# mayataka/idocp

Measured on AMD Instinct MI355X. Metric: SQP iterations/sec (whole node), higher is better.
Workload: dtype f64; 1 GPU; ANYmal OCPSolver N=100 T=5.05 FP64, trotting contact sequence (1 lift + 9 impulse events, 120 stages incl. impulse / aux / lift stages, switching constraints; BASELINE.json configs[2]); batch=1024 independent OCP instances per GPU, replicas across GPUs; horizon=100, batch_per_gpu=1024, parallelism=replicas x1

## Files before the change

idocp_amd/csrc/ocp_condense_kernel.hip:

```cpp
#include <hip/hip_runtime.h>

#include <cstdlib>

#include "dev_dense.hpp"
#include "dev_lie.hpp"
#include "dev_rnea_tangent.hpp"
#include "ocp_device.hpp"
#include "ocp_launch.hpp"

namespace idocp_dev {

#ifdef IDOCP_K5_TILES16
#define K5_TILE_PAIR mfmaTilePairTN
#else
#define K5_TILE_PAIR mfmaTilePairTN4
#endif

__device__ __forceinline__ double ocpLimit(const OcpProblem* __restrict__ P, int comp, int r) {
  switch (comp) {
    case 0: return P->q_min[r];
    case 1: return P->q_max[r];
    case 2: return -P->v_max[r];
    case 3: return P->v_max[r];
    case 4: return -P->u_max[r];
// ... 464 lines not shown
        for (int m = 0; m < 6; ++m) acc += sm[S::BL + r + SF * m] * sm[GG + c + SF * m];
#pragma unroll
        for (int m = 0; m < NJ; ++m) acc += sm[TT + r + SF * m] * sm[S::JM + c + SF * (6 + m)];
        sm[S::SM + r + SF * c] = acc;
      }
      waveLdsSync();
      if (dimf > 0) {
        constexpr int WW = (TT + SF * NJ + SF * SF <= S::VEC) ? TT + SF * NJ : S::WSM;
        static_assert(WW != S::WSM || !S::SEP_MINV, "the narrow layouts keep W behind G and Jl D^-1");
        spdInverseCholDpp<SF>(&sm[S::SM], SF, dimf, lane, &s_ok, &sm[WW], SF);
      }
    } else {
      ldsFlagWait(&s_gt, 1, lane);
      ldsFlagWait(&s_ba, 3, lane);
      for (int e = lane; e < dimf * NJ; e += 64) {
        const int c = e / dimfd, r = e - c * dimfd;
        double acc = sm[TT + r + SF * c];
#pragma unroll
        for (int m = 0; m < 6; ++m) acc += sm[GG + r + SF * m] * sm[S::MINV + m + NV * (6 + c)];
        sm[S::BL + r + SF * (6 + c)] = acc;
      }
    }
    STAMPW(3);
  }
  blockLdsBarrier();
  STAMP(2);
  if (MERIT) {
    rneaAssembleNominal<D>(tid, sc, out);
    blockLdsBarrier();
    if (!impulse && tid >= 6 && tid < NV && nd->has_u) sm[S::IDC + tid] -= s_g[L::S_U + tid - 6];
    blockLdsBarrier();
    if (tid < dimvf) merit_viol += dt * fabs(sm[S::IDC + tid]);
    if (sw_dimi > 0 && tid >= 200 && tid < 200 + sw_dimi) merit_viol += fabs(B.swc[rec * L::SWC + L::W_P + tid - 200]);
    blockLdsBarrier();
    sm[S::ERR + tid] = merit_cost; sm[S::ERR + nt + tid] = merit_viol;
    blockLdsBarrier();
    if (tid < 2) {
      double e = 0.0;
      for (int t = 0; t < nt; ++t) e += sm[S::ERR + nt * tid + t];
      if (B.ext) e += B.ext[rec * L::EXT + (tid == 1 ? L::X_VIOL : L::X_COST)];
      B.merit_stage[rec * 4 + tid] = e;
    }
    return;
  }
  STAMP(5);
  asm volatile("" : "+v"(tid) :: "memory");
  if (RESIDUAL) {
    rneaAssembleQV<D>(bwp, tid, nt, sc, out);
    blockLdsBarrier();
    if (!impulse && tid >= 6 && tid < NV && nd->has_u) sm[S::IDC + tid] -= s_g[L::S_U + tid - 6];
    blockLdsBarrier();
    if (tid >= 128 && tid < 128 + NV) {
      const int r = tid - 128;
      const double dq = dotAny(&sm[S::DIDC + SVF * r], 1, &sm[S::BM], 1, dimvf);
      const double dv = dotAny(&sm[S::DIDC + SVF * (NV + r)], 1, &sm[S::BM], 1, dimvf);
      const double da = dotAny(&sm[S::MM + NV * r], 1, &sm[S::BM], 1, NV) + dotAny(&sm[S::JM + SF * r], 1, &sm[S::BM + NV], 1, dimf);
      const double lq = sm[S::LQ + r] + dt * dq, lv = sm[S::LV + r] + dt * dv, la = sm[S::LA + r] + dt * da;
      const double idr = sm[S::IDC + r];
      err_local += lq * lq + lv * lv + la * la + dt * dt * idr * idr;
    } else if (tid >= 192 && tid < 192 + NC) {
      const int c = tid - 192;
      if (nd->active[c]) {
        const int row = nd->row_of[c];
        for (int x = 0; x < 3; ++x) {
          double jb = 0.0;
          for (int col = 0; col < NV; ++col) jb += sm[S::JM + (row + x) + SF * col] * sm[S::BM + col];
          const double lf = sm[S::LF + row + x] - dt * jb;
          const double cr = sm[S::IDC + NV + row + x];
          err_local += lf * lf + dt * dt * cr * cr;
        }
      }
    }
    if (sw_dimi > 0 && tid >= 200 && tid < 200 + sw_dimi) {
      const double pr = B.swc[rec * L::SWC + L::W_P + tid - 200];
      err_local += pr * pr;
    }
    blockLdsBarrier();
    sm[S::ERR + tid] = err_local + (BWD ? 1.0 : dt * dt) * err_ipm;
    blockLdsBarrier();
    if (tid == 0) {
      double e = 0.0;
      for (int t = 0; t < nt; ++t) e += sm[S::ERR + t];
      if (B.ext) e += (BWD ? 1.0 : dt * dt) * B.ext[rec * L::EXT + L::X_ERR];
      B.err_stage[rec] = e;
    }
    return;
  }
  constexpr bool EARLY_MJ = (SVF * SVF <= RS::FEET);
  auto assembleTR = [&]() {
    for (int e = tid; e < dimf * NV; e += nt) {
      const int c = e / NV, r = e - c * NV;
      const double tr = dotAny(&sm[S::BL + SF * r], 1, &sm[S::SM + SF * c], 1, dimf);
      sm[S::MJ + r + SVF * (NV + c)] = tr;
      sm[S::MJ + (NV + c) + SVF * r] = tr;
    }
    for (int e = tid; e < dimf * dimf; e += nt) { const int c = e / dimfd, r = e - c * dimfd; sm[S::MJ + (NV + r) + SVF * (NV + c)] = -sm[S::SM + r + SF * c]; }
  };
  STAMPW(7);
  rneaAssembleQV<D>(bwp, tid, nt, sc, out);
  STAMPW(5);
  if (tid >= 160 && tid < 160 + NV) sm[S::LA + tid - 160] += dt * sm[S::TLA + tid - 160];
  if (tid >= 128 && tid < 128 + 6) {
    const int r = tid - 128;
    double acc = 0.0;
    for (int m2 = 0; m2 < 6; ++m2) acc += sm[S::FQQI + r + 6 * m2] * sm[S::FQ + m2];
    sm[S::FQ6 + r] = BWD ? acc : -acc;
  }
  if constexpr (EARLY_MJ) assembleTR();
  STAMPW(6);
  blockLdsBarrier();
  if (tid < dimvf) {
    double val = sm[S::IDC + tid];
    if (!impulse && tid >= 6 && tid < NV && nd->has_u) { val -= s_g[L::S_U + tid - 6]; sm[S::IDC + tid] = val; }
    sm[S::DIDC + tid + SVF * NX] = val;
  }
  if (tid >= 64 && tid < 64 + 6) sm[S::FQ + tid - 64] = sm[S::FQ6 + tid - 64];
  if constexpr (!EARLY_MJ) {
    assembleTR();
    blockLdsBarrier();
  }
  STAMP(6);
  for (int e = tid; e < NV * NV; e += nt) {
    const int c = e / NV, r = e - c * NV;
    sm[S::MJ + r + SVF * c] = sm[S::MINV + e] - dotAny(&sm[S::MJ + r + SVF * NV], SVF, &sm[S::BL + SF * c], 1, dimf);
  }
  {
    const int part = tid & 3;
    double acc = 0.0;
    int dst = -1;
    double sgn = dt;
    if (tid < 4 * NX) {
      const int g = tid >> 2;
      const int q4 = (dimvf + 3) >> 2, k0 = part * q4, k1 = (k0 + q4 < dimvf) ? k0 + q4 : dimvf;
      const double* col = &sm[S::DIDC + SVF * g];
      for (int k = k0; k < k1; ++k) acc += col[k] * sm[S::BM + k];
      dst = (g < NV) ? S::LQ + g : S::LV + g - NV;
    } else if (tid >= 160 && tid < 160 + 4 * SF) {
      const int r = (tid - 160) >> 2;
      if (r < dimf) {
        constexpr int q4 = (NV + 3) / 4;
        const int k0 = part * q4, k1 = (k0 + q4 < NV) ? k0 + q4 : NV;
        for (int col = k0; col < k1; ++col) acc += sm[S::JM + r + SF * col] * sm[S::BM + col];
        dst = S::LF + r; sgn = -dt;
      }
    }
    acc += __shfl_xor(acc, 1);
    acc += __shfl_xor(acc, 2);
    if (part == 0 && dst >= 0) sm[dst] += sgn * acc;
  }
  blockLdsBarrier();

  const double hu = (PLAIN || nd->has_u) ? 1.0 : 0.0;
  STAMP(7);
  {
    const int wave = tid >> 6, lane = tid & 63;
    constexpr int TX = (NX + 15) / 16;
    static_assert(RVF <= 32, "two row tiles");
    for (int jb = wave; jb < TX; jb += nt >> 6) {
      mfma_d4 a0, a1;
      const int r1 = dimvf > 16 ? dimvf - 16 : 1;
      K5_TILE_PAIR<RVF>(&sm[S::MJ], dimvf < 16 ? dimvf : 16, &sm[S::DIDC + SVF * 16 * jb], NX + 1 - 16 * jb, &sm[S::MJ + SVF * 16], r1,
                          &sm[S::DIDC + SVF * 16 * jb], NX + 1 - 16 * jb, SVF, SVF, dimvf, lane, a0, a1);
      auto put = [&](int r, int c, double v) { sm[S::MJD + r + SVF * c] = v; };
      mfmaTileStore(a0, 0, 16 * jb, dimvf, NX + 1, lane, put);
      mfmaTileStore(a1, 16, 16 * jb, dimvf, NX + 1, lane, put);
    }
  }
  STAMP(11);
  const double* const mjidc = &sm[S::MJD + SVF * NX];
#pragma unroll
  for (int t = 0; t < (NV * NV + nt - 1) / nt; ++t) {
    const int e = tid + nt * t;
    if (e < NV * NV) { const int c = e / NV, r = e - c * NV; sm[S::QAFU + r + SVF * c] = hu * sm[S::QAA + r] * sm[S::MJ + r + SVF * c]; }
  }
  for (int e = tid; e < dimf * NV; e += nt) {
    const int c = e / dimfd, r = e - c * dimfd;
    sm[S::QAFU + NV + r + SVF * c] = hu * dotAny(&sm[S::QFF + r], SF, &sm[S::MJ + NV + SVF * c], 1, dimf);
  }
  STAMP(12);
  blockLdsBarrier();
  STAMP(13);
#pragma unroll
  for (int t = 0; t < (NV * NX + nt - 1) / nt; ++t) {
    const int e = tid + nt * t;
    if (e < NV * NX) { const int c = e / NV, r = e - c * NV; sm[S::QAFQV + r + SVF * c] = -sm[S::QAA + r] * sm[S::MJD + r + SVF * c]; }
  }
  for (int e = tid; e < dimf * NX; e += nt) {
    const int c = e / dimfd, r = e - c * dimfd;
    sm[S::QAFQV + NV + r + SVF * c] = -dotAny(&sm[S::QFF + r], SF, &sm[S::MJD + NV + SVF * c], 1, dimf);
  }
  if (tid < dimvf) {
    const int r = tid;
    double val;
    if (r < NV) val = sm[S::LA + r] - sm[S::QAA + r] * mjidc[r];
    else { double acc = 0.0; for (int p = 0; p < dimf; ++p) acc += sm[S::QFF + (r - NV) + SF * p] * mjidc[NV + p]; val = -sm[S::LF + r - NV] - acc; }
    sm[S::LAF + r] = val;
  }
  blockLdsBarrier();
  STAMP(8);
  {
    const int wave = tid >> 6, lane = tid & 63;
    constexpr int NJOB = 14;
    static_assert(NX <= 48 && NV <= 32 && NU <= 16, "tile counts of the job list");
    auto operands = [&](int j, const double*& X, int& xr, const double*& Y, int& yc, int& r0, int& c0) {
      if (j < 6) {
        const int ib = j < 3 ? 0 : (j < 5 ? 1 : 2), jb = j < 3 ? j : (j < 5 ? j - 2 : 2);
        X = &sm[S::MJD + SVF * 16 * ib]; xr = NX - 16 * ib; Y = &sm[S::QAFQV + SVF * 16 * jb]; yc = NX - 16 * jb; r0 = 16 * ib; c0 = 16 * jb;
      } else if (j < 12) {
        const int ib = (j - 6) >> 1, jb = (j - 6) & 1;
        X = &sm[S::MJD + SVF * 16 * ib]; xr = NX - 16 * ib; Y = &sm[S::QAFU + SVF * 16 * jb]; yc = NV - 16 * jb; r0 = 16 * ib; c0 = 16 * jb;
      } else {
        const int ib = j - 12;
        X = &sm[S::MJ + SVF * 16 * ib]; xr = NV - 16 * ib; Y = &sm[S::QAFU + SVF * 6]; yc = NU; r0 = 16 * ib; c0 = 0;
      }
    };
    auto finish = [&](int j, const mfma_d4& acc, int r0, int c0) {
      const int r = r0 + (lane & 15), g4 = lane >> 4;
      if (j < 6) {
        double b6[4];
        const double dg = sm[S::HQD + (r < NX ? r : NX - 1)];
        static_assert(S::HVD == S::HQD + NV, "one diagonal vector");
#pragma unroll
        for (int q = 0; q < 4; ++q) { const int c = c0 + g4 + 4 * q; b6[q] = sm[S::QB6 + (r < 6 ? r : 5) + 6 * (c < 6 ? c : 5)]; }
#pragma unroll
        for (int q = 0; q < 4; ++q) {
          const int c = c0 + g4 + 4 * q;
          const double base = (r < 6 && c < 6) ? b6[q] : (r == c ? dg : 0.0);
          if (r <= c && c < NX) kk[L::K_QXX + L::xsym(r, c)] = base - acc[q];
        }
      } else if (j < 12) {
#pragma unroll
        for (int q = 0; q < 4; ++q) {
          const int c = c0 + g4 + 4 * q;
          double* dst = c < 6 ? ee + (L::E_QXUP + r + NX * c) : kk + (L::K_QXU + r + NX * (c - 6));
          if (r < NX && c < NV) *dst = -acc[q];
        }
      } else {
        double hd[4];
#pragma unroll
        for (int q = 0; q < 4; ++q) { const int c = c0 + g4 + 4 * q; hd[q] = sm[S::HUD + (c < NU ? c : NU - 1)]; }
#pragma unroll
        for (int q = 0; q < 4; ++q) {
          const int c = c0 + g4 + 4 * q;
          double* dst = r < 6 ? ee + (L::E_QUUP + r + 6 * c) : kk + (L::K_QUU + (r - 6) + NU * c);
          const double v = acc[q] + ((r >= 6 && r - 6 == c) ? hd[q] : 0.0);
          if (r < NV && c < NU) *dst = v;
        }
      }
    };
    auto pair = [&](auto jc) {
      constexpr int j = decltype(jc)::value;
      const double *X0, *Y0, *X1, *Y1;
      int xr0, yc0, r00, c00, xr1, yc1, r01, c01;
      operands(j, X0, xr0, Y0, yc0, r00, c00);
      operands(j + 1, X1, xr1, Y1, yc1, r01, c01);
      mfma_d4 a0, a1;
      K5_TILE_PAIR<RVF>(X0, xr0, Y0, yc0, X1, xr1, Y1, yc1, SVF, SVF, dimvf, lane, a0, a1);
      finish(j, a0, r00, c00);
      finish(j + 1, a1, r01, c01);
    };
    static_assert(nt == 256 && NJOB == 14, "four wavefronts: jobs 2 w, 2 w + 1 and 2 w + 8, 2 w + 9");
    switch (__builtin_amdgcn_readfirstlane(wave)) {
      case 0: pair(std::integral_constant<int, 0>{}); pair(std::integral_constant<int, 8>{}); break;
      case 1: pair(std::integral_constant<int, 2>{}); pair(std::integral_constant<int, 10>{}); break;
      case 2: pair(std::integral_constant<int, 4>{}); pair(std::integral_constant<int, 12>{}); break;
      default: pair(std::integral_constant<int, 6>{}); break;
    }
  }
  STAMP(14);
  {
    const int part = tid & 3, g = tid >> 2;
    const int q4 = (dimvf + 3) >> 2, k0 = part * q4, k1 = (k0 + q4 < dimvf) ? k0 + q4 : dimvf;
    double acc = 0.0;
    if (g < NX) { const double* col = &sm[S::MJD + SVF * g]; for (int k = k0; k < k1; ++k) acc += col[k] * sm[S::LAF + k]; }
    else if (g < NX + NV) { const double* row = &sm[S::MJ + (g - NX)]; for (int k = k0; k < k1; ++k) acc += row[SVF * k] * sm[S::LAF + k]; }
    acc += __shfl_xor(acc, 1);
    acc += __shfl_xor(acc, 2);
    if (part == 0) {
      if (g < NV) sm[S::LQ + g] -= acc;
      else if (g < NX) sm[S::LV + g - NV] -= acc;
      else if (g < NX + NV) {
        const int r = g - NX;
        if (r < 6) sm[S::LUP + r] += hu * acc; else sm[S::LU + r - 6] += hu * acc;
        sm[S::FV + r] -= dt * mjidc[r];
      }
    }
  }
  static_assert(4 * (NX + NV) <= nt, "a quad per row of the vector updates");
  blockLdsBarrier();

  STAMP(9);
  typedef double wd2 __attribute__((ext_vector_type(2)));
  static_assert(NV % 2 == 0 && SVF % 2 == 0 && S::MJD % 2 == 0 && L::K_FVQ % 2 == 0 && L::K_FVV % 2 == 0 && L::KKT % 2 == 0, "16-byte stores of Fvq / Fvv");
  for (int e = tid; e < NV * NV / 2; e += nt) {
    const int c = e / (NV / 2), r = 2 * (e - c * (NV / 2));
    const wd2 mq = *reinterpret_cast<const wd2*>(&sm[S::MJD + r + SVF * c]), mvv = *reinterpret_cast<const wd2*>(&sm[S::MJD + r + SVF * (NV + c)]);
    const double one = BWD ? -1.0 : 1.0;
    wd2 fq, fv;
    fq.x = -dt * mq.x; fq.y = -dt * mq.y;
    fv.x = -dt * mvv.x + (r == c ? one : 0.0); fv.y = -dt * mvv.y + (r + 1 == c ? one : 0.0);
    *reinterpret_cast<wd2*>(&kk[L::K_FVQ + r + NV * c]) = fq;
    *reinterpret_cast<wd2*>(&kk[L::K_FVV + r + NV * c]) = fv;
  }
  for (int e = tid; e < NV * NU; e += nt) { const int c = e / NV, r = e - c * NV; kk[L::K_FVU + e] = hu * dt * sm[S::MJ + r + SVF * (6 + c)]; }
  if (tid < NV) {
    kk[L::K_LX + tid] = sm[S::LQ + tid]; kk[L::K_LX + NV + tid] = sm[S::LV + tid];
    kk[L::K_FX + tid] = sm[S::FQ + tid]; kk[L::K_FX + NV + tid] = sm[S::FV + tid];
  }
  if (tid < NU) kk[L::K_LU + tid] = sm[S::LU + tid];
  for (int t = tid; t < RVF * (RVF + 1) / 2; t += nt) {
    const int pr = t / (RVF + 1), idx = t - pr * (RVF + 1);
    const bool lo = idx <= pr;
    const int r = lo ? pr : RVF - 1 - pr, c = lo ? idx : idx - pr - 1;
    ee[L::E_MJ + r * (r + 1) / 2 + c] = sm[S::MJ + r + SVF * c];
  }
  static_assert(RVF % 2 == 0 && NVF % 2 == 0 && L::E_MJD % 2 == 0 && L::EXP % 2 == 0, "16-byte stores of MJtJinv_dIDCdqv");
  for (int e = tid; e < (RVF / 2) * NX; e += nt) {
    const int c = e / (RVF / 2), r = 2 * (e - c * (RVF / 2));
    *reinterpret_cast<wd2*>(&ee[L::E_MJD + r + NVF * c]) = *reinterpret_cast<const wd2*>(&sm[S::MJD + r + SVF * c]);
  }
  if (tid < NV) ee[L::E_QAA + tid] = sm[S::QAA + tid];
  for (int e = tid; e < SF * SF; e += nt) { const int c = e / SF, r = e - c * SF; ee[L::E_QFF + r + NF * c] = sm[S::QFF + e]; }
  if (tid < RVF) { ee[L::E_MJIDC + tid] = mjidc[tid]; ee[L::E_LAF + tid] = sm[S::LAF + tid]; }
  if (tid < 6) ee[L::E_LUP + tid] = sm[S::LUP + tid];
  if (sw_dimi > 0) {
    const int dimi = sw_dimi;
    double* __restrict__ W = B.swc + rec * L::SWC;
    for (int e = tid; e < dimi * NX; e += nt) {
      const int c = e / dimi, j = e - c * dimi;
      double acc = 0.0;
      for (int m2 = 0; m2 < NV; ++m2) acc += W[L::W_PHIA + j + NF * m2] * sm[S::MJD + m2 + SVF * c];
      W[L::W_PHIX + j + NF * c] -= acc;
    }
    for (int e = tid; e < dimi * NU; e += nt) {
      const int c = e / dimi, j = e - c * dimi;
      double acc = 0.0;
      for (int m2 = 0; m2 < NV; ++m2) acc += W[L::W_PHIA + j + NF * m2] * sm[S::MJ + m2 + SVF * (6 + c)];
      W[L::W_PHIU + j + NF * c] = acc;
    }
    if (tid < dimi) {
      double acc = 0.0;
      for (int m2 = 0; m2 < NV; ++m2) acc += W[L::W_PHIA + tid + NF * m2] * mjidc[m2];
      W[L::W_P + tid] -= acc;
    }
  }
  STAMP(10);
  if (tid == 0 && !s_ok && B.status[b] == 0) B.status[b] = 1 + pos;
  };
  stage((long)blockIdx.x);
#undef STAMP
#undef STAMPW
}


template <typename D>
__global__ __launch_bounds__(64) void parnmpc_lie_kernel(OcpBuffers B, const double* __restrict__ q0) {
  using L = OcpLayout<D>;
  constexpr int NQ = D::NQ;
  const OcpProblem* __restrict__ P = B.prob;
  const int M = B.M;
  const long unit = (long)blockIdx.x * 64 + threadIdx.x;
  if (unit >= (long)P->batch * (M - 1)) return;
  const long b = unit / (M - 1);
  const int pos = (int)(unit - b * (M - 1));
  const OcpNode* __restrict__ nd = B.nodes + pos;
  const int task = blockIdx.y;
  const long rec = b * B.NS + nd->slot;
  const double* __restrict__ s = B.sol + rec * L::SOL;
  const double* __restrict__ q = s + L::S_Q;
  double* __restrict__ zz = B.lie + rec * L::LIE;
  double R[9], p[3], Ja[36], Jb[36], d6[6];
  if (task == 0) {
    lieRelative(B.q_ref + (long)pos * NQ, q, R, p);
    lieLog6(R, p, d6);
    lieJlog6(R, p, Ja);
    for (int k = 0; k < 36; ++k) zz[L::Z_JQ + k] = Ja[k];
    for (int k = 0; k < 6; ++k) zz[L::Z_QDIFF + k] = d6[k];
  } else if (task == 1) {
    lieRelative(B.sol + (b * B.NS + nd->next) * L::SOL + L::S_Q, q, R, p);
    lieJlog6(R, p, Ja);
    for (int k = 0; k < 36; ++k) zz[L::Z_FQQ + k] = Ja[k];
  } else {
    const double* __restrict__ q_prev = (nd->prev < 0) ? (q0 + b * NQ) : (B.sol + (b * B.NS + nd->prev) * L::SOL + L::S_Q);
    lieRelative(q, q_prev, R, p);
    lieLog6(R, p, d6);
    for (int k = 0; k < 6; ++k) zz[L::Z_FQ6 + k] = d6[k];
    lieJlog6(R, p, Ja);
    lieDDiffArg0(R, p, Ja, Jb);
    for (int k = 0; k < 36; ++k) zz[L::Z_FQQP + k] = Jb[k];
    lieBlockInverse(Ja, Jb);
    for (int k = 0; k < 36; ++k) zz[L::Z_FQQI + k] = Jb[k];
  }
}

template <typename D>
static void launchCondense(const OcpBuffers& B, long batch, int M, int dimf, const double* q0, hipStream_t st, bool residual, int part = 0) {
  const size_t smem = CondenseSmem<D>::TOTAL * sizeof(double);
  static bool configured = false;
  if (!configured) {
    (void)hipFuncSetAttribute((const void*)ocp_condense_kernel<D, false, -1>, hipFuncAttributeMaxDynamicSharedMemorySize, (int)smem);
    (void)hipFuncSetAttribute((const void*)ocp_condense_kernel<D, false, -1, false, false, true>, hipFuncAttributeMaxDynamicSharedMemorySize, (int)smem);
    (void)hipFuncSetAttribute((const void*)ocp_condense_kernel<D, false, D::NF>, hipFuncAttributeMaxDynamicSharedMemorySize, (int)smem);
    (void)hipFuncSetAttribute((const void*)ocp_condense_kernel<D, false, D::NF, false, false, true>, hipFuncAttributeMaxDynamicSharedMemorySize, (int)smem);
    (void)hipFuncSetAttribute((const void*)ocp_condense_kernel<D, true, -1>, hipFuncAttributeMaxDynamicSharedMemorySize, (int)smem);
    configured = true;
  }
  const unsigned blocks = (unsigned)(batch * M);
  if (part != 2) {
    OcpLaunch<D>::nominal(B, batch, M, st, q0);
    OcpLaunch<D>::extRows(B, batch, M, residual, st);
  }
  if (part == 1) return;
  if (residual) hipLaunchKernelGGL((ocp_condense_kernel<D, true, -1>), dim3(blocks), dim3(256), smem, st, B, q0);
  else if (dimf == D::NF) { if (B.leg_axes_xyy) hipLaunchKernelGGL((ocp_condense_kernel<D, false, D::NF, false, false, true>), dim3(blocks), dim3(256), smem, st, B, q0); else hipLaunchKernelGGL((ocp_condense_kernel<D, false, D::NF>), dim3(blocks), dim3(256), smem, st, B, q0); }
  else { if (B.leg_axes_xyy) hipLaunchKernelGGL((ocp_condense_kernel<D, false, -1, false, false, true>), dim3(blocks), dim3(256), smem, st, B, q0); else hipLaunchKernelGGL((ocp_condense_kernel<D, false, -1>), dim3(blocks), dim3(256), smem, st, B, q0); }
  if (!residual) OcpLaunch<D>::extHessian(B, batch, M, st);
}

template <typename D>
void OcpLaunch<D>::condense(const OcpBuffers& B, long batch, int M, int dimf, const double* q0, hipStream_t st, int part) {
  launchCondense<D>(B, batch, M, dimf, q0, st, false, part);
}
template <typename D>
void OcpLaunch<D>::condenseMixed(const OcpBuffers& B, long batch, int M, const int n[5], const double* q0, hipStream_t st, int part, hipStream_t st_imp) {
  const size_t smem = CondenseSmem<D>::TOTAL * sizeof(double), smem_half = CondenseSmem<D, D::NF / 2>::TOTAL * sizeof(double);
  static bool configured = false;
  if (!configured) {
    (void)hipFuncSetAttribute((const void*)ocp_condense_kernel<D, false, -1>, hipFuncAttributeMaxDynamicSharedMemorySize, (int)smem);
    (void)hipFuncSetAttribute((const void*)ocp_condense_kernel<D, false, -1, false, false, true>, hipFuncAttributeMaxDynamicSharedMemorySize, (int)smem);
    (void)hipFuncSetAttribute((const void*)ocp_condense_kernel<D, false, D::NF>, hipFuncAttributeMaxDynamicSharedMemorySize, (int)smem);
    (void)hipFuncSetAttribute((const void*)ocp_condense_kernel<D, false, D::NF, false, false, true>, hipFuncAttributeMaxDynamicSharedMemorySize, (int)smem);
    (void)hipFuncSetAttribute((const void*)ocp_condense_kernel<D, false, D::NF / 2>, hipFuncAttributeMaxDynamicSharedMemorySize, (int)smem_half);
    (void)hipFuncSetAttribute((const void*)ocp_condense_kernel<D, false, D::NF / 2, false, false, true>, hipFuncAttributeMaxDynamicSharedMemorySize, (int)smem_half);
    (void)hipFuncSetAttribute((const void*)ocp_condense_kernel<D, false, D::NF / 2, false, false, false, true>, hipFuncAttributeMaxDynamicSharedMemorySize, (int)smem_half);
    (void)hipFuncSetAttribute((const void*)ocp_condense_kernel<D, false, 0>, hipFuncAttributeMaxDynamicSharedMemorySize, (int)smem_half);
    (void)hipFuncSetAttribute((const void*)ocp_condense_kernel<D, false, 0, false, false, true>, hipFuncAttributeMaxDynamicSharedMemorySize, (int)smem_half);
    (void)hipFuncSetAttribute((const void*)ocp_condense_kernel<D, false, D::NF / 2, false, false, true, true>, hipFuncAttributeMaxDynamicSharedMemorySize, (int)smem_half);
    configured = true;
  }
  const unsigned blocks = (unsigned)(batch * M);
  const double* none = nullptr;
  if (part != 2) {
    OcpLaunch<D>::nominal(B, batch, M, st, q0, st_imp);
    OcpLaunch<D>::extRows(B, batch, M, false, st);
  }
  if (part == 1) return;
  if (part == 5) { OcpLaunch<D>::extHessian(B, batch, M, st); return; }
  const bool big = part != 4, rest = part != 3;
  if (big && n[1] > 0) { if (B.leg_axes_xyy) hipLaunchKernelGGL((ocp_condense_kernel<D, false, D::NF / 2, false, false, true>), dim3((unsigned)(batch * n[1])), dim3(256), smem_half, st, B, q0, none, B.cond_pos + n[0], n[1]); else hipLaunchKernelGGL((ocp_condense_kernel<D, false, D::NF / 2>), dim3((unsigned)(batch * n[1])), dim3(256), smem_half, st, B, q0, none, B.cond_pos + n[0], n[1]); }
  if (rest && n[0] > 0) { if (B.leg_axes_xyy) hipLaunchKernelGGL((ocp_condense_kernel<D, false, D::NF, false, false, true>), dim3((unsigned)(batch * n[0])), dim3(256), smem, st, B, q0, none, B.cond_pos, n[0]); else hipLaunchKernelGGL((ocp_condense_kernel<D, false, D::NF>), dim3((unsigned)(batch * n[0])), dim3(256), smem, st, B, q0, none, B.cond_pos, n[0]); }
  if (rest && n[4] > 0) { if (B.leg_axes_xyy) hipLaunchKernelGGL((ocp_condense_kernel<D, false, 0, false, false, true>), dim3((unsigned)(batch * n[4])), dim3(256), smem_half, st, B, q0, none, B.cond_pos + n[0] + n[1] + n[2] + n[3], n[4]); else hipLaunchKernelGGL((ocp_condense_kernel<D, false, 0>), dim3((unsigned)(batch * n[4])), dim3(256), smem_half, st, B, q0, none, B.cond_pos + n[0] + n[1] + n[2] + n[3], n[4]); }
  if (rest && n[3] > 0) { if (B.leg_axes_xyy) hipLaunchKernelGGL((ocp_condense_kernel<D, false, D::NF / 2, false, false, true, true>), dim3((unsigned)(batch * n[3])), dim3(256), smem_half, st, B, q0, none, B.cond_pos + n[0] + n[1] + n[2], n[3]); else hipLaunchKernelGGL((ocp_condense_kernel<D, false, D::NF / 2, false, false, false, true>), dim3((unsigned)(batch * n[3])), dim3(256), smem_half, st, B, q0, none, B.cond_pos + n[0] + n[1] + n[2], n[3]); }
  if (rest && n[2] > 0) { if (B.leg_axes_xyy) hipLaunchKernelGGL((ocp_condense_kernel<D, false, -1, false, false, true>), dim3((unsigned)(batch * n[2])), dim3(256), smem, st, B, q0, none, B.cond_pos + n[0] + n[1], n[2]); else hipLaunchKernelGGL((ocp_condense_kernel<D, false, -1>), dim3((unsigned)(batch * n[2])), dim3(256), smem, st, B, q0, none, B.cond_pos + n[0] + n[1], n[2]); }
  if (part == 0 || part == 2) OcpLaunch<D>::extHessian(B, batch, M, st);
}
template <typename D>
void OcpLaunch<D>::merit(const OcpBuffers& Btry, long batch, int M, const double* q0, hipStream_t st) {
  const size_t smem = CondenseSmem<D>::TOTAL * sizeof(double);
  static bool configured = false;
  if (!configured) {
    (void)hipFuncSetAttribute((const void*)ocp_condense_kernel<D, true, -1, false, true>, hipFuncAttributeMaxDynamicSharedMemorySize, (int)smem);
    configured = true;
  }
  const unsigned blocks = (unsigned)(batch * M);
  OcpLaunch<D>::nominal(Btry, batch, M, st, q0);
  OcpLaunch<D>::extRows(Btry, batch, M, true, st);
  hipLaunchKernelGGL((ocp_condense_kernel<D, true, -1, false, true>), dim3(blocks), dim3(256), smem, st, Btry, q0);
}
template <typename D>
void OcpLaunch<D>::meritBackwardEuler(const OcpBuffers& Btry, long batch, int M, const double* q0, const double* v0, hipStream_t st) {
  const size_t smem = CondenseSmem<D>::TOTAL * sizeof(double);
  static bool configured = false;
  if (!configured) {
    (void)hipFuncSetAttribute((const void*)ocp_condense_kernel<D, true, -1, true, true>, hipFuncAttributeMaxDynamicSharedMemorySize, (int)smem);
    configured = true;
  }
  const unsigned stages = (unsigned)(batch * (M - 1));
// ... 38 lines not shown
```

idocp_amd/csrc/dev_dense.hpp:

```cpp
#ifndef IDOCP_DEV_DENSE_HPP_
#define IDOCP_DEV_DENSE_HPP_

#include <hip/hip_runtime.h>

#include <type_traits>

namespace idocp_dev {

struct MatView {
  double* p; int rs, cs;
  __device__ __forceinline__ double& operator()(int i, int j) const { return p[i * rs + j * cs]; }
};
__device__ __forceinline__ MatView colMajor(double* p, int ld) { return MatView{p, 1, ld}; }
__device__ __forceinline__ MatView transposed(MatView a) { return MatView{a.p, a.cs, a.rs}; }
__device__ __forceinline__ MatView sub(MatView a, int i0, int j0) { return MatView{a.p + i0 * a.rs + j0 * a.cs, a.rs, a.cs}; }

template <int U>
__device__ __forceinline__ double dotStrided(const double* a, int as, const double* b, int bs, int k) {
  double acc[U];
#pragma unroll
  for (int u = 0; u < U; ++u) acc[u] = 0.0;
  for (int p = 0; p < k; p += U) {
#pragma unroll
    for (int u = 0; u < U; ++u) acc[u] += a[(p + u) * as] * b[(p + u) * bs];
  }
  double r = acc[0];
#pragma unroll
  for (int u = 1; u < U; ++u) r += acc[u];
  return r;
}
__device__ __forceinline__ double dotAny(const double* a, int as, const double* b, int bs, int k) {
  if (k % 6 == 0) return dotStrided<6>(a, as, b, bs, k);
  if (k % 3 == 0) return dotStrided<3>(a, as, b, bs, k);
  return dotStrided<1>(a, as, b, bs, k);
}
__device__ __forceinline__ void mm(MatView C, MatView A, MatView Bm, int m, int n, int k, double alpha, bool accumulate,
                                   int tid, int nthreads) {
  for (int e = tid; e < m * n; e += nthreads) {
    const int j = e / m, i = e - j * m;
    const double acc = dotAny(A.p + i * A.rs, A.cs, Bm.p + j * Bm.cs, Bm.rs, k);
    if (accumulate) C(i, j) += alpha * acc; else C(i, j) = alpha * acc;
  }
}

__device__ __forceinline__ void mv(double* y, MatView A, const double* x, int m, int k, double alpha, bool accumulate, int tid,
                                   int nthreads) {
  for (int i = tid; i < m; i += nthreads) {
    const double acc = dotAny(A.p + i * A.rs, A.cs, x, 1, k);
    if (accumulate) y[i] += alpha * acc; else y[i] = alpha * acc;
  }
}

__device__ __forceinline__ void spdInverse(double* A, double* W, int ld, int n, int tid, int nthreads, int* ok) {
  const int e0 = tid, e1 = tid + nthreads;
  const bool has0 = e0 < n * n, has1 = e1 < n * n;
  const int j0 = has0 ? e0 / n : 0, i0 = has0 ? e0 - j0 * n : 0;
  const int j1 = has1 ? e1 / n : 0, i1 = has1 ? e1 - j1 * n : 0;
  double* src = A;
  double* dst = W;
  __syncthreads();
  for (int k = 0; k < n; ++k) {
    const double p = src[k + k * ld];
    if (tid == 0 && !(p > 0.0)) *ok = 0;
    const double ip = 1.0 / p;
    if (has0) {
      const double aik = src[i0 + k * ld], akj = src[k + j0 * ld], aij = src[i0 + j0 * ld];
      dst[i0 + j0 * ld] = (i0 == k) ? ((j0 == k) ? ip : akj * ip) : ((j0 == k) ? -aik * ip : aij - aik * akj * ip);
    }
    if (has1) {
      const double aik = src[i1 + k * ld], akj = src[k + j1 * ld], aij = src[i1 + j1 * ld];
      dst[i1 + j1 * ld] = (i1 == k) ? ((j1 == k) ? ip : akj * ip) : ((j1 == k) ? -aik * ip : aij - aik * akj * ip);
    }
    __syncthreads();
    double* t = src; src = dst; dst = t;
  }
  if (src != A) {
    if (has0) A[i0 + j0 * ld] = src[i0 + j0 * ld];
    if (has1) A[i1 + j1 * ld] = src[i1 + j1 * ld];
    __syncthreads();
  }
}

template <int ME>
__device__ __forceinline__ void spdInverseWave(double* A, double* W, int ld, int n, int lane, int* ok) {
  int ii[ME], jj[ME];
#pragma unroll
  for (int t = 0; t < ME; ++t) { const int e = lane + 64 * t; const int j = e / n; jj[t] = j; ii[t] = e - j * n; }
  double* src = A;
  double* dst = W;
  for (int k = 0; k < n; ++k) {
    const double p = src[k + k * ld];
    if (lane == 0 && !(p > 0.0)) *ok = 0;
    const double ip = 1.0 / p;
#pragma unroll
    for (int t = 0; t < ME; ++t) {
      if (lane + 64 * t < n * n) {
        const int i = ii[t], j = jj[t];
        const double aik = src[i + k * ld], akj = src[k + j * ld], aij = src[i + j * ld];
        dst[i + j * ld] = (i == k) ? ((j == k) ? ip : akj * ip) : ((j == k) ? -aik * ip : aij - aik * akj * ip);
      }
    }
    __builtin_amdgcn_fence(__ATOMIC_SEQ_CST, "wavefront");
    __builtin_amdgcn_wave_barrier();
    double* tmp = src; src = dst; dst = tmp;
  }
  if (src != A) {
#pragma unroll
    for (int t = 0; t < ME; ++t) if (lane + 64 * t < n * n) A[ii[t] + jj[t] * ld] = src[ii[t] + jj[t] * ld];
    __builtin_amdgcn_fence(__ATOMIC_SEQ_CST, "wavefront");
    __builtin_amdgcn_wave_barrier();
  }
}

__device__ __forceinline__ double readLaneF64(double v, int lane) {
  const int lo = __builtin_amdgcn_readlane(__double2loint(v), lane), hi = __builtin_amdgcn_readlane(__double2hiint(v), lane);
  return __hiloint2double(hi, lo);
}
__device__ __forceinline__ double recipNewton(double p) {
  double x = __builtin_amdgcn_rcp(p);
  double e = __builtin_fma(-p, x, 1.0);
  x = __builtin_fma(x, e, x);
  e = __builtin_fma(-p, x, 1.0);
  return __builtin_fma(x, e, x);
}
template <int N>
__device__ __forceinline__ void spdInverseRows(double* A, int ld, int n, int lane, int* ok) {
  double a[N];
  const bool on = lane < n;
#pragma unroll
  for (int j = 0; j < N; ++j) a[j] = (on && j < n) ? A[lane + ld * j] : 0.0;
#pragma unroll
  for (int k = 0; k < N; ++k) {
    if (k < n) {
      double prow[N];
#pragma unroll
      for (int j = 0; j < N; ++j) prow[j] = readLaneF64(a[j], k);
      const double p = prow[k];
      if (lane == 0 && !(p > 0.0)) *ok = 0;
      const double ip = recipNewton(p);
      const double aik = a[k];
      const bool isk = lane == k;
#pragma unroll
      for (int j = 0; j < N; ++j) {
        if (j == k) continue;
        const double akj = prow[j];
        a[j] = isk ? akj * ip : a[j] - aik * akj * ip;
      }
      a[k] = isk ? ip : -aik * ip;
    }
  }
#pragma unroll
  for (int j = 0; j < N; ++j) if (on && j < n) A[lane + ld * j] = a[j];
}

__device__ __forceinline__ void rsqrtNewton(double p, double& rs, double& s) {
  double x = __builtin_amdgcn_rsq(p);
  double e = __builtin_fma(-p * x, x, 1.0);
  x = __builtin_fma(0.5 * x, e, x);
  e = __builtin_fma(-p * x, x, 1.0);
  x = __builtin_fma(0.5 * x, e, x);
  double sq = p * x;
  const double r = __builtin_fma(-sq, sq, p);
  sq = __builtin_fma(r, 0.5 * x, sq);
  rs = x; s = sq;
}

template <int LANE>
__device__ __forceinline__ double rowBcast(double v) {
  int lo = __double2loint(v), hi = __double2hiint(v);
  lo = __builtin_amdgcn_update_dpp(0, lo, 0x150 + LANE, 0xF, 0xF, true);
  hi = __builtin_amdgcn_update_dpp(0, hi, 0x150 + LANE, 0xF, 0xF, true);
  return __hiloint2double(hi, lo);
}
__device__ __forceinline__ double rowBcastN(double v, int n) {
  switch (n) {
    case 0: return rowBcast<0>(v);   case 1: return rowBcast<1>(v);   case 2: return rowBcast<2>(v);   case 3: return rowBcast<3>(v);
    case 4: return rowBcast<4>(v);   case 5: return rowBcast<5>(v);   case 6: return rowBcast<6>(v);   case 7: return rowBcast<7>(v);
    case 8: return rowBcast<8>(v);   case 9: return rowBcast<9>(v);   case 10: return rowBcast<10>(v); case 11: return rowBcast<11>(v);
// ... 540 lines not shown
```

Before: 220,400 SQP iterations/s.

## Fuse Qafqv/Laf into MFMA tile wavefronts and drop two block barriers

Each MFMA wavefront now computes the Qafqv entries and the force rows for its own column tile right after storing MJD, using only a wavefront-level LDS sync. The otherwise idle wavefront computes Qafu concurrently. The vector updates now write straight to the global KKT/expansion buffers instead of updating LDS and copying afterwards. Together these remove two block-wide barriers. In exchange the work is spread unevenly across wavefronts, and correctness depends on the dropped barrier (LU/FV/LUP no longer being read from LDS afterwards) and on fp contraction being off so rounding is preserved.

Result: no change. 220,000 SQP iterations/s, median of 4 (-0.2%).

```diff
diff --git a/idocp_amd/csrc/ocp_condense_kernel.hip b/idocp_amd/csrc/ocp_condense_kernel.hip
--- a/idocp_amd/csrc/ocp_condense_kernel.hip
+++ b/idocp_amd/csrc/ocp_condense_kernel.hip
@@ -640,50 +640,49 @@
 
   const double hu = (PLAIN || nd->has_u) ? 1.0 : 0.0;
   STAMP(7);
+  const double* const mjidc = &sm[S::MJD + SVF * NX];
   {
     const int wave = tid >> 6, lane = tid & 63;
     constexpr int TX = (NX + 15) / 16;
     static_assert(RVF <= 32, "two row tiles");
-    for (int jb = wave; jb < TX; jb += nt >> 6) {
+    static_assert(TX < nt / 64, "one pair per wavefront, and a wavefront left for Qafu_full");
+    if (wave < TX) {
+      const int jb = wave;
       mfma_d4 a0, a1;
       const int r1 = dimvf > 16 ? dimvf - 16 : 1;
       K5_TILE_PAIR<RVF>(&sm[S::MJ], dimvf < 16 ? dimvf : 16, &sm[S::DIDC + SVF * 16 * jb], NX + 1 - 16 * jb, &sm[S::MJ + SVF * 16], r1,
                           &sm[S::DIDC + SVF * 16 * jb], NX + 1 - 16 * jb, SVF, SVF, dimvf, lane, a0, a1);
-      auto put = [&](int r, int c, double v) { sm[S::MJD + r + SVF * c] = v; };
+      auto put = [&](int r, int c, double v) {
+        sm[S::MJD + r + SVF * c] = v;
+        if (r < NV && c < NX) sm[S::QAFQV + r + SVF * c] = -sm[S::QAA + r] * v;
+      };
       mfmaTileStore(a0, 0, 16 * jb, dimvf, NX + 1, lane, put);
       mfmaTileStore(a1, 16, 16 * jb, dimvf, NX + 1, lane, put);
+      waveLdsSync();
+      const int cw = (NX - 16 * jb < 16) ? NX - 16 * jb : 16;
+      for (int e = lane; e < dimf * cw; e += 64) {
+        const int c = 16 * jb + e / dimfd, r = e - (e / dimfd) * dimfd;
+        sm[S::QAFQV + NV + r + SVF * c] = -dotAny(&sm[S::QFF + r], SF, &sm[S::MJD + NV + SVF * c], 1, dimf);
+      }
+      if (jb == NX / 16 && lane < dimvf) {
+        const int r = lane;
+        double val;
+        if (r < NV) val = sm[S::LA + r] - sm[S::QAA + r] * mjidc[r];
+        else { double acc = 0.0; for (int p = 0; p < dimf; ++p) acc += sm[S::QFF + (r - NV) + SF * p] * mjidc[NV + p]; val = -sm[S::LF + r - NV] - acc; }
+        sm[S::LAF + r] = val;
+      }
+    } else {
+      constexpr int nq = nt - 64 * TX;
+      const int t0 = tid - 64 * TX;
+      for (int e = t0; e < NV * NV; e += nq) { const int c = e / NV, r = e - c * NV; sm[S::QAFU + r + SVF * c] = hu * sm[S::QAA + r] * sm[S::MJ + r + SVF * c]; }
+      for (int e = t0; e < dimf * NV; e += nq) {
+        const int c = e / dimfd, r = e - c * dimfd;
+        sm[S::QAFU + NV + r + SVF * c] = hu * dotAny(&sm[S::QFF + r], SF, &sm[S::MJ + NV + SVF * c], 1, dimf);
+      }
     }
   }
   STAMP(11);
-  const double* const mjidc = &sm[S::MJD + SVF * NX];
-#pragma unroll
-  for (int t = 0; t < (NV * NV + nt - 1) / nt; ++t) {
-    const int e = tid + nt * t;
-    if (e < NV * NV) { const int c = e / NV, r = e - c * NV; sm[S::QAFU + r + SVF * c] = hu * sm[S::QAA + r] * sm[S::MJ + r + SVF * c]; }
-  }
-  for (int e = tid; e < dimf * NV; e += nt) {
-    const int c = e / dimfd, r = e - c * dimfd;
-    sm[S::QAFU + NV + r + SVF * c] = hu * dotAny(&sm[S::QFF + r], SF, &sm[S::MJ + NV + SVF * c], 1, dimf);
-  }
   STAMP(12);
-  blockLdsBarrier();
-  STAMP(13);
-#pragma unroll
-  for (int t = 0; t < (NV * NX + nt - 1) / nt; ++t) {
-    const int e = tid + nt * t;
-    if (e < NV * NX) { const int c = e / NV, r = e - c * NV; sm[S::QAFQV + r + SVF * c] = -sm[S::QAA + r] * sm[S::MJD + r + SVF * c]; }
-  }
-  for (int e = tid; e < dimf * NX; e += nt) {
-    const int c = e / dimfd, r = e - c * dimfd;
-    sm[S::QAFQV + NV + r + SVF * c] = -dotAny(&sm[S::QFF + r], SF, &sm[S::MJD + NV + SVF * c], 1, dimf);
-  }
-  if (tid < dimvf) {
-    const int r = tid;
-    double val;
-    if (r < NV) val = sm[S::LA + r] - sm[S::QAA + r] * mjidc[r];
-    else { double acc = 0.0; for (int p = 0; p < dimf; ++p) acc += sm[S::QFF + (r - NV) + SF * p] * mjidc[NV + p]; val = -sm[S::LF + r - NV] - acc; }
-    sm[S::LAF + r] = val;
-  }
   blockLdsBarrier();
   STAMP(8);
   {
@@ -765,17 +764,17 @@
     acc += __shfl_xor(acc, 1);
     acc += __shfl_xor(acc, 2);
     if (part == 0) {
-      if (g < NV) sm[S::LQ + g] -= acc;
-      else if (g < NX) sm[S::LV + g - NV] -= acc;
+#pragma clang fp contract(off)
+      if (g < NV) kk[L::K_LX + g] = sm[S::LQ + g] - acc;
+      else if (g < NX) kk[L::K_LX + g] = sm[S::LV + g - NV] - acc;
       else if (g < NX + NV) {
         const int r = g - NX;
-        if (r < 6) sm[S::LUP + r] += hu * acc; else sm[S::LU + r - 6] += hu * acc;
-        sm[S::FV + r] -= dt * mjidc[r];
+        if (r < 6) ee[L::E_LUP + r] = sm[S::LUP + r] + hu * acc; else kk[L::K_LU + r - 6] = sm[S::LU + r - 6] + hu * acc;
+        kk[L::K_FX + NV + r] = sm[S::FV + r] - dt * mjidc[r];
       }
     }
   }
   static_assert(4 * (NX + NV) <= nt, "a quad per row of the vector updates");
-  blockLdsBarrier();
 
   STAMP(9);
   typedef double wd2 __attribute__((ext_vector_type(2)));
@@ -791,11 +790,7 @@
     *reinterpret_cast<wd2*>(&kk[L::K_FVV + r + NV * c]) = fv;
   }
   for (int e = tid; e < NV * NU; e += nt) { const int c = e / NV, r = e - c * NV; kk[L::K_FVU + e] = hu * dt * sm[S::MJ + r + SVF * (6 + c)]; }
-  if (tid < NV) {
-    kk[L::K_LX + tid] = sm[S::LQ + tid]; kk[L::K_LX + NV + tid] = sm[S::LV + tid];
-    kk[L::K_FX + tid] = sm[S::FQ + tid]; kk[L::K_FX + NV + tid] = sm[S::FV + tid];
-  }
-  if (tid < NU) kk[L::K_LU + tid] = sm[S::LU + tid];
+  if (tid < NV) kk[L::K_FX + tid] = sm[S::FQ + tid];
   for (int t = tid; t < RVF * (RVF + 1) / 2; t += nt) {
     const int pr = t / (RVF + 1), idx = t - pr * (RVF + 1);
     const bool lo = idx <= pr;
@@ -810,7 +805,6 @@
   if (tid < NV) ee[L::E_QAA + tid] = sm[S::QAA + tid];
   for (int e = tid; e < SF * SF; e += nt) { const int c = e / SF, r = e - c * SF; ee[L::E_QFF + r + NF * c] = sm[S::QFF + e]; }
   if (tid < RVF) { ee[L::E_MJIDC + tid] = mjidc[tid]; ee[L::E_LAF + tid] = sm[S::LAF + tid]; }
-  if (tid < 6) ee[L::E_LUP + tid] = sm[S::LUP + tid];
   if (sw_dimi > 0) {
     const int dimi = sw_dimi;
     double* __restrict__ W = B.swc + rec * L::SWC;
```

## Fuse MJD tile epilogue with Qafqv products and early global stores

Applied to the files above, without the earlier changes.

For the plain trotting stage specialization (6 contact dims, NV=18), the MFMA product MJtJinv*dIDC is consumed directly from registers. The same waves compute the -Qaa*MJD rows, the contact rows of Qafqv, the LAF vector, and the Fvq/Fvv/MJD global stores. The spare waves compute Qafu, Fvu and the packed MJ stores concurrently. This removes one block-wide LDS barrier and several separate passes that re-read MJD from LDS. In exchange it adds code specialization and per-wave syncs, and the global stores become less coalesced (scalar instead of 16-byte).

New measurement: 217,900 SQP iterations/s before, 216,100 SQP iterations/s after. Within noise of the previous version (-0.8%).

```diff
diff --git a/idocp_amd/csrc/dev_dense.hpp b/idocp_amd/csrc/dev_dense.hpp
--- a/idocp_amd/csrc/dev_dense.hpp
+++ b/idocp_amd/csrc/dev_dense.hpp
@@ -24,6 +24,18 @@
 #pragma unroll
     for (int u = 0; u < U; ++u) acc[u] += a[(p + u) * as] * b[(p + u) * bs];
   }
+  double r = acc[0];
+#pragma unroll
+  for (int u = 1; u < U; ++u) r += acc[u];
+  return r;
+}
+template <int U, typename FA, typename FB>
+__device__ __forceinline__ double dotRegs(FA a, FB b) {
+  double acc[U];
+#pragma unroll
+  for (int u = 0; u < U; ++u) acc[u] = 0.0;
+#pragma unroll
+  for (int u = 0; u < U; ++u) acc[u] += a(u) * b(u);
   double r = acc[0];
 #pragma unroll
   for (int u = 1; u < U; ++u) r += acc[u];
diff --git a/idocp_amd/csrc/ocp_condense_kernel.hip b/idocp_amd/csrc/ocp_condense_kernel.hip
--- a/idocp_amd/csrc/ocp_condense_kernel.hip
+++ b/idocp_amd/csrc/ocp_condense_kernel.hip
@@ -640,6 +640,94 @@
 
   const double hu = (PLAIN || nd->has_u) ? 1.0 : 0.0;
   STAMP(7);
+#ifdef IDOCP_K5_OLD_BACKHALF
+  constexpr bool REG_BACK = false;
+#else
+  constexpr bool REG_BACK = PLAIN && !RESIDUAL && !MERIT && !BWD && DIMF == 6 && NV == 18 && NX == 36 && std::is_same<D, LeggedDims<4, 3>>::value;
+#endif
+#ifdef IDOCP_K5_LATE_STORES
+  constexpr bool EARLY_ST = false;
+#else
+  constexpr bool EARLY_ST = REG_BACK;
+#endif
+  if constexpr (REG_BACK) {
+    const int wv = __builtin_amdgcn_readfirstlane(tid >> 6), lane = tid & 63;
+    constexpr int TX = (NX + 15) / 16;
+    static_assert(TX <= 3 && RVF > 16 && RVF <= 32 && NX / 16 == TX - 1 && NX % 16 != 0, "three column blocks, [ID; C] in the last one; two row tiles");
+    if (wv < TX) {
+      const int jb = wv;
+      mfma_d4 a0, a1;
+      K5_TILE_PAIR<RVF>(&sm[S::MJ], 16, &sm[S::DIDC + SVF * 16 * jb], NX + 1 - 16 * jb, &sm[S::MJ + SVF * 16], RVF - 16,
+                          &sm[S::DIDC + SVF * 16 * jb], NX + 1 - 16 * jb, SVF, SVF, dimvf, lane, a0, a1);
+      const int li = lane & 15, g4 = lane >> 4;
+      const bool lo1 = li < RVF - 16, ac1 = li < NV - 16;
+      const double qa0 = sm[S::QAA + li], qa1 = sm[S::QAA + (ac1 ? 16 + li : NV - 1)];
+      const double one = 1.0;
+#pragma unroll
+      for (int q = 0; q < 4; ++q) {
+        const int c = 16 * jb + g4 + 4 * q;
+        if (16 * jb + 4 * q >= NX + 1) continue;
+        const double m0 = a0[q], m1 = a1[q];
+        if (c < NX + 1) { sm[S::MJD + li + SVF * c] = m0; if (lo1) sm[S::MJD + 16 + li + SVF * c] = m1; }
+        if (c < NX) {
+          sm[S::QAFQV + li + SVF * c] = -qa0 * m0;
+          if (ac1) sm[S::QAFQV + 16 + li + SVF * c] = -qa1 * m1;
+          if constexpr (EARLY_ST) {
+            ee[L::E_MJD + li + NVF * c] = m0;
+            if (lo1) ee[L::E_MJD + 16 + li + NVF * c] = m1;
+            const bool isq = c < NV;
+            const int cv = isq ? c : c - NV;
+            double* fdst = kk + (isq ? L::K_FVQ : L::K_FVV) + NV * cv;
+            const double f0 = isq ? -dt * m0 : -dt * m0 + (li == cv ? one : 0.0);
+            const double f1 = isq ? -dt * m1 : -dt * m1 + (16 + li == cv ? one : 0.0);
+            fdst[li] = f0;
+            if (ac1) fdst[16 + li] = f1;
+          }
+        }
+      }
+      waveLdsSync();
+      {
+        typedef double cd2 __attribute__((ext_vector_type(2)));
+        static_assert(SF == 6 && S::QFF % 2 == 0 && (S::MJD + NV) % 2 == 0 && (S::QAFQV + NV) % 2 == 0 && SVF % 2 == 0, "16-byte pieces of the contact rows");
+        const int c = 16 * jb + li, rp = 2 * g4;
+        if (g4 < SF / 2 && c < NX) {
+          double mj[SF];
+          cd2 qf[SF];
+#pragma unroll
+          for (int p = 0; p < SF; p += 2) { const cd2 t = *reinterpret_cast<const cd2*>(&sm[S::MJD + NV + p + SVF * c]); mj[p] = t.x; mj[p + 1] = t.y; }
+#pragma unroll
+          for (int p = 0; p < SF; ++p) qf[p] = *reinterpret_cast<const cd2*>(&sm[S::QFF + rp + SF * p]);
+          cd2 res;
+          res.x = -dotRegs<SF>([&](int p) { return qf[p].x; }, [&](int p) { return mj[p]; });
+          res.y = -dotRegs<SF>([&](int p) { return qf[p].y; }, [&](int p) { return mj[p]; });
+          *reinterpret_cast<cd2*>(&sm[S::QAFQV + NV + rp + SVF * c]) = res;
+        }
+      }
+      if (jb == TX - 1 && lane < dimvf) {
+        const double* const mjidc = &sm[S::MJD + SVF * NX];
+        const int r = lane;
+        double val;
+        if (r < NV) val = sm[S::LA + r] - sm[S::QAA + r] * mjidc[r];
+        else { double acc = 0.0; for (int p = 0; p < dimf; ++p) acc += sm[S::QFF + (r - NV) + SF * p] * mjidc[NV + p]; val = -sm[S::LF + r - NV] - acc; }
+        sm[S::LAF + r] = val;
+      }
+    } else {
+      for (int e = lane; e < NV * NV; e += 64) { const int c = e / NV, r = e - c * NV; sm[S::QAFU + r + SVF * c] = hu * sm[S::QAA + r] * sm[S::MJ + r + SVF * c]; }
+      for (int e = lane; e < dimf * NV; e += 64) {
+        const int c = e / dimfd, r = e - c * dimfd;
+        sm[S::QAFU + NV + r + SVF * c] = hu * dotAny(&sm[S::QFF + r], SF, &sm[S::MJ + NV + SVF * c], 1, dimf);
+      }
+      if constexpr (EARLY_ST) {
+      for (int e = lane; e < NV * NU; e += 64) { const int c = e / NV, r = e - c * NV; kk[L::K_FVU + e] = hu * dt * sm[S::MJ + r + SVF * (6 + c)]; }
+      for (int t = lane; t < RVF * (RVF + 1) / 2; t += 64) {
+        const int pr = t / (RVF + 1), idx = t - pr * (RVF + 1);
+        const bool lo = idx <= pr;
+        const int r = lo ? pr : RVF - 1 - pr, c = lo ? idx : idx - pr - 1;
+        ee[L::E_MJ + r * (r + 1) / 2 + c] = sm[S::MJ + r + SVF * c];
+      }
+      }
+    }
+  } else
   {
     const int wave = tid >> 6, lane = tid & 63;
     constexpr int TX = (NX + 15) / 16;
@@ -656,6 +744,7 @@
   }
   STAMP(11);
   const double* const mjidc = &sm[S::MJD + SVF * NX];
+  if constexpr (!REG_BACK) {
 #pragma unroll
   for (int t = 0; t < (NV * NV + nt - 1) / nt; ++t) {
     const int e = tid + nt * t;
@@ -665,9 +754,11 @@
     const int c = e / dimfd, r = e - c * dimfd;
     sm[S::QAFU + NV + r + SVF * c] = hu * dotAny(&sm[S::QFF + r], SF, &sm[S::MJ + NV + SVF * c], 1, dimf);
   }
+  }
   STAMP(12);
   blockLdsBarrier();
   STAMP(13);
+  if constexpr (!REG_BACK) {
 #pragma unroll
   for (int t = 0; t < (NV * NX + nt - 1) / nt; ++t) {
     const int e = tid + nt * t;
@@ -685,6 +776,7 @@
     sm[S::LAF + r] = val;
   }
   blockLdsBarrier();
+  }
   STAMP(8);
   {
     const int wave = tid >> 6, lane = tid & 63;
@@ -780,6 +872,7 @@
   STAMP(9);
   typedef double wd2 __attribute__((ext_vector_type(2)));
   static_assert(NV % 2 == 0 && SVF % 2 == 0 && S::MJD % 2 == 0 && L::K_FVQ % 2 == 0 && L::K_FVV % 2 == 0 && L::KKT % 2 == 0, "16-byte stores of Fvq / Fvv");
+  if constexpr (!EARLY_ST) {
   for (int e = tid; e < NV * NV / 2; e += nt) {
     const int c = e / (NV / 2), r = 2 * (e - c * (NV / 2));
     const wd2 mq = *reinterpret_cast<const wd2*>(&sm[S::MJD + r + SVF * c]), mvv = *reinterpret_cast<const wd2*>(&sm[S::MJD + r + SVF * (NV + c)]);
@@ -791,21 +884,24 @@
     *reinterpret_cast<wd2*>(&kk[L::K_FVV + r + NV * c]) = fv;
   }
   for (int e = tid; e < NV * NU; e += nt) { const int c = e / NV, r = e - c * NV; kk[L::K_FVU + e] = hu * dt * sm[S::MJ + r + SVF * (6 + c)]; }
+  }
   if (tid < NV) {
     kk[L::K_LX + tid] = sm[S::LQ + tid]; kk[L::K_LX + NV + tid] = sm[S::LV + tid];
     kk[L::K_FX + tid] = sm[S::FQ + tid]; kk[L::K_FX + NV + tid] = sm[S::FV + tid];
   }
   if (tid < NU) kk[L::K_LU + tid] = sm[S::LU + tid];
+  static_assert(RVF % 2 == 0 && NVF % 2 == 0 && L::E_MJD % 2 == 0 && L::EXP % 2 == 0, "16-byte stores of MJtJinv_dIDCdqv");
+  if constexpr (!EARLY_ST) {
   for (int t = tid; t < RVF * (RVF + 1) / 2; t += nt) {
     const int pr = t / (RVF + 1), idx = t - pr * (RVF + 1);
     const bool lo = idx <= pr;
     const int r = lo ? pr : RVF - 1 - pr, c = lo ? idx : idx - pr - 1;
     ee[L::E_MJ + r * (r + 1) / 2 + c] = sm[S::MJ + r + SVF * c];
   }
-  static_assert(RVF % 2 == 0 && NVF % 2 == 0 && L::E_MJD % 2 == 0 && L::EXP % 2 == 0, "16-byte stores of MJtJinv_dIDCdqv");
   for (int e = tid; e < (RVF / 2) * NX; e += nt) {
     const int c = e / (RVF / 2), r = 2 * (e - c * (RVF / 2));
     *reinterpret_cast<wd2*>(&ee[L::E_MJD + r + NVF * c]) = *reinterpret_cast<const wd2*>(&sm[S::MJD + r + SVF * c]);
+  }
   }
   if (tid < NV) ee[L::E_QAA + tid] = sm[S::QAA + tid];
   for (int e = tid; e < SF * SF; e += nt) { const int c = e / SF, r = e - c * SF; ee[L::E_QFF + r + NF * c] = sm[S::QFF + e]; }
```
